# secondlaw-ai/skyrim

Hardware: AMD Instinct MI355X
Metric: 6-h forecast steps/sec on 721x1440 state, 1/2/4/8 MI355X; per-channel max rel-err vs ref (higher is better)
Workload: dtype f16; 1 GPU; Pangu 6-h autoregressive rollout, 721x1440x69 state (13 levels x 5 vars + 4 surface), random-init weights (64 M params), state resident in HBM, 1 ensemble membe; parallelism=single GPU, members=1, finite=True, rounding=compensated, term_plan=0x66f

## Files before the change

skyrim_amd/csrc/attention.hip:

```cpp
#include <cstdlib>
#include "gemm_dma.h"
#include "launchers.h"

namespace skp {

__device__ __forceinline__ int attn_key(int f, int row) {
    return f < 8 ? 32 * (f >> 1) + 8 * (row >> 2) + 4 * (f & 1) + (row & 3) : 128 + row;
}

__device__ __forceinline__ void attn_softmax_pv(f32x4 (&s)[9], const uint4 (&vf)[2][5], f32x4 (&o)[2], f32x4& osum) {
    typedef f16 T;
    const float LOG2E = 1.4426950408889634f;
    float mx = s[0][0];
#pragma unroll
    for (int f = 0; f < 9; ++f)
#pragma unroll
        for (int r = 0; r < 4; ++r) mx = fmaxf(mx, s[f][r]);
    mx = fmaxf(mx, __shfl_xor(mx, 16));
    mx = fmaxf(mx, __shfl_xor(mx, 32));
    const float mxl = mx * LOG2E;
#pragma unroll
    for (int f = 0; f < 9; ++f)
#pragma unroll
        for (int r = 0; r < 4; ++r) s[f][r] = __builtin_amdgcn_exp2f(__builtin_fmaf(s[f][r], LOG2E, -mxl));
    o[0] = f32x4{0.f, 0.f, 0.f, 0.f}; o[1] = f32x4{0.f, 0.f, 0.f, 0.f}; osum = f32x4{0.f, 0.f, 0.f, 0.f};
    const uint4 ones = make_uint4(0x3C003C00u, 0x3C003C00u, 0x3C003C00u, 0x3C003C00u);
#pragma unroll
    for (int kb = 0; kb < 5; ++kb) {
        float pv[8];
#pragma unroll
        for (int r = 0; r < 4; ++r) {
            pv[r] = s[2 * kb][r];
            pv[4 + r] = (kb < 4) ? s[(2 * kb + 1) % 9][r] : 0.f;
        }
        uint4 pf[1];
        split8<T, 1>(pv, pf);
#pragma unroll
        for (int df = 0; df < 2; ++df) o[df] = OpT<T>::mfma(as_v8<T>(vf[df][kb]), as_v8<T>(pf[0]), o[df]);
        osum = OpT<T>::mfma(as_v8<T>(ones), as_v8<T>(pf[0]), osum);
    }
}

constexpr int BT_ROW = 28, BT_COPY = 144 * BT_ROW + 120;

template <class TO, int NPL_O>
__global__ void __launch_bounds__(256) __attribute__((amdgpu_waves_per_eu(3, 3))) earth_attention2_kernel(const f16* __restrict__ q, const f16* __restrict__ k,
                                                              const f16* __restrict__ vt, const f16* __restrict__ bias_cmp, TO* __restrict__ out,
                                                              long long out_plane, int ld_out, int nW, int heads) {
    typedef f16 T;
    __shared__ __attribute__((aligned(16))) f16 tabs[4 * BT_COPY];
    const int lane = threadIdx.x & 63, wave = threadIdx.x >> 6;
    const int th = blockIdx.x;
    const int head = th % heads, type = th / heads;
    const int l15 = lane & 15, g = lane >> 4;
    {
        const f16* src = bias_cmp + (long long)th * 3456;
        for (int i = threadIdx.x; i < 3456; i += 256) {
            const int r = i / 24, e = i - 24 * r;
            const f16 v = src[i];
            if (e < 23) {
#pragma unroll
                for (int c = 0; c < 4; ++c) tabs[c * BT_COPY + r * BT_ROW + e + c] = v;
            }
        }
    }
    int koff[9];
#pragma unroll
    for (int f = 0; f < 9; ++f) {
        const int k0 = f < 8 ? 32 * (f >> 1) + 8 * g + 4 * (f & 1) : 128 + 4 * g;
        const int zk = k0 / 72, hk = (k0 / 12) % 6, wk0 = k0 % 12;
        koff[f] = 2 * ((2 * zk * 36 + 6 * hk) * BT_ROW + wk0);
    }
    __syncthreads();
    const char* tb = reinterpret_cast<const char*>(tabs);

    for (int wi = wave; wi < nW; wi += 4) {
        const int win = type * nW + wi;
        const long long base = (long long)win * heads + head;
        const T* qp = q + base * (WIN_TOKENS * HEAD_DIM) + l15 * HEAD_DIM + g * 8;
        const T* kp = k + base * (WIN_TOKENS * HEAD_DIM) + g * 8;
        const T* vp = vt + base * (WIN_TOKENS * HEAD_DIM) + (8 * (l15 >> 2) + (l15 & 3)) * WIN_TOKENS;

        uint4 kf[9];
#pragma unroll
        for (int f = 0; f < 9; ++f) kf[f] = *reinterpret_cast<const uint4*>(kp + attn_key(f, l15) * HEAD_DIM);
        uint4 vf[2][5];
#pragma unroll
        for (int df = 0; df < 2; ++df)
#pragma unroll
            for (int kb = 0; kb < 5; ++kb) {
                const T* s = vp + df * 4 * WIN_TOKENS;
                if (kb < 4) vf[df][kb] = *reinterpret_cast<const uint4*>(s + kb * 32 + g * 8);
                else { const uint2 lo = *reinterpret_cast<const uint2*>(s + 128 + g * 4); vf[df][kb] = make_uint4(lo.x, lo.y, 0, 0); }
            }
        uint4 qn = *reinterpret_cast<const uint4*>(qp);
#pragma unroll 1
        for (int qf = 0; qf < 9; ++qf) {
            const uint4 qv = qn;
            if (qf < 8) qn = *reinterpret_cast<const uint4*>(qp + (qf + 1) * 16 * HEAD_DIM);
            const int qi = 16 * qf + l15;
            const int zq = qi >= 72 ? 1 : 0, hq = (qi - 72 * zq) / 12, wq = qi - 72 * zq - 12 * hq;
            const int c = (wq + 1) & 3;
            const char* bq = tb + 2 * (c * BT_COPY + (zq * 36 + hq) * BT_ROW + (11 - wq) + c);
            uint2 bias[9];
#pragma unroll
            for (int f = 0; f < 9; ++f) bias[f] = *reinterpret_cast<const uint2*>(bq + koff[f]);

            f32x4 s[9];
#pragma unroll
            for (int f = 0; f < 9; ++f) {
                typedef f16 h4 __attribute__((ext_vector_type(4)));
                const h4 b = __builtin_bit_cast(h4, bias[f]);
                s[f] = OpT<T>::mfma(as_v8<T>(kf[f]), as_v8<T>(qv), f32x4{(float)b[0], (float)b[1], (float)b[2], (float)b[3]});
            }
            f32x4 o[2], osum;
            attn_softmax_pv(s, vf, o, osum);
            const float inv = __builtin_amdgcn_rcpf(osum[0]);
            TO* orow = out + blk_off((long long)win * WIN_TOKENS + qf * 16 + l15, head * HEAD_DIM, ld_out) + g * 8;
            const float y[8] = {o[0][0] * inv, o[0][1] * inv, o[0][2] * inv, o[0][3] * inv, o[1][0] * inv, o[1][1] * inv, o[1][2] * inv, o[1][3] * inv};
            store8_planes<TO, NPL_O>(orow, out_plane, y);
        }
    }
}


template <int C_, int PL_>
struct QaShape {
    static constexpr int C = C_, PL = PL_, KS = C / 32, NWAVES = 8, THREADS = 64 * NWAVES;
    static constexpr int BLK_KIB = KS * 2 * PL;
    static constexpr int W_BYTES = 3 * BLK_KIB * 1024;
    static constexpr int TAB_BYTES = (4 * BT_COPY * 2 + 1023) / 1024 * 1024;
    static constexpr int RING_BYTES = 6 * 1024;
    static constexpr int SMEM = W_BYTES + TAB_BYTES + 1024 + NWAVES * RING_BYTES;
    static_assert(SMEM <= 160 * 1024, "LDS");
};

struct QkvAttnArgs {
    const f16* xs;
    const int* widx;
    const f16* wf;
    const float* bias;
    const f16* bias_cmp;
    const f16* zrow;
    f16* out; long long out_plane;
    int nW, heads, types;
    float scale;
};

template <class S, int NPL_O>
__global__ void __launch_bounds__(S::THREADS) __attribute__((amdgpu_waves_per_eu(2, 2)))
qkv_attention_kernel(const QkvAttnArgs a) {
    typedef f16 T;
    constexpr int C = S::C, KS = S::KS, PL = S::PL;
    extern __shared__ __attribute__((aligned(16))) char smem[];
    char* wl = smem;
    f16* tabs = reinterpret_cast<f16*>(smem + S::W_BYTES);
    float* qb = reinterpret_cast<float*>(smem + S::W_BYTES + S::TAB_BYTES);
    const int tid = threadIdx.x, lane = tid & 63, l15 = lane & 15, g = lane >> 4;
    const int wave = __builtin_amdgcn_readfirstlane(tid >> 6);
    const int xcd = blockIdx.x & 7, slot = blockIdx.x >> 3;
    const int head = slot % a.heads, type = xcd + 8 * (slot / a.heads);
    if (type >= a.types) return;
    const int th = type * a.heads + head;
    {
        const unsigned lds_base = (unsigned)(size_t)smem;
#pragma unroll
        for (int which = 0; which < 3; ++which) {
            const f16* src = a.wf + ((long long)(which * a.heads + head) * S::BLK_KIB << 9) + lane * 8;
            for (int p = wave; p < S::BLK_KIB; p += S::NWAVES) glds16(src + (p << 9), lds_base + (unsigned)((which * S::BLK_KIB + p) << 10));
        }
        const f16* src = a.bias_cmp + (long long)th * 3456;
        constexpr int NT = (3456 + S::THREADS - 1) / S::THREADS;
        f16 tv[NT];
#pragma unroll
        for (int j = 0; j < NT; ++j) { const int i = tid + j * S::THREADS; tv[j] = src[i < 3456 ? i : 0]; }
#pragma unroll
        for (int j = 0; j < NT; ++j) {
            const int i = tid + j * S::THREADS;
            const int r = i / 24, e = i - 24 * r;
            if (i < 3456 && e < 23) {
#pragma unroll
                for (int c = 0; c < 4; ++c) tabs[c * BT_COPY + r * BT_ROW + e + c] = tv[j];
            }
        }
        if (tid < 96) qb[tid] = a.bias[(tid >> 5) * C + head * HEAD_DIM + (tid & 31)];
    }
    int koff[9];
#pragma unroll
    for (int f = 0; f < 9; ++f) {
        const int k0 = f < 8 ? 32 * (f >> 1) + 8 * g + 4 * (f & 1) : 128 + 4 * g;
        const int zk = k0 / 72, hk = (k0 / 12) % 6, wk0 = k0 % 12;
        koff[f] = 2 * ((2 * zk * 36 + 6 * hk) * BT_ROW + wk0);
    }
    int srcn[9];
    auto load_src = [&](int wi_) {
        const int w_ = type * a.nW + wi_;
#pragma unroll
        for (int f = 0; f < 9; ++f) srcn[f] = a.widx[w_ * WIN_TOKENS + attn_key(f, l15)];
    };
    load_src(wave < a.nW ? wave : 0);
    asm volatile("s_waitcnt vmcnt(0)" ::: "memory");
    __syncthreads();
    const char* tb = reinterpret_cast<const char*>(tabs);
    const char* wrd = wl + lane * 16;
    const unsigned ring_base = (unsigned)(size_t)smem + (unsigned)(S::W_BYTES + S::TAB_BYTES + 1024 + wave * S::RING_BYTES);
    const char* ring_rd = smem + S::W_BYTES + S::TAB_BYTES + 1024 + wave * S::RING_BYTES + lane * 16;

    for (int wi = wave; wi < a.nW; wi += S::NWAVES) {
        const int win = type * a.nW + wi;
        int src[9];
#pragma unroll
        for (int f = 0; f < 9; ++f) src[f] = srcn[f];
        uint4 qv[9], kf[9];
        uint2 vh[9][2];
        const T* xp[3];
        int xstep[3];
        auto point = [&](int tg_) {
#pragma unroll
            for (int i = 0; i < 3; ++i) {
                const int r = src[3 * tg_ + i];
                xp[i] = r >= 0 ? a.xs + blk_off(r, g * 8, C) : a.zrow;
                xstep[i] = r >= 0 ? 512 : 0;
            }
        };
        auto fetch = [&](int ks) {
#pragma unroll
            for (int i = 0; i < 3; ++i) glds16(xp[i] + ks * xstep[i], ring_base + (unsigned)(((ks & 1) * 3 + i) << 10));
        };
        point(0);
        fetch(0);
        fetch(1);
#pragma unroll
        for (int tg = 0; tg < 3; ++tg) {
            f32x4 qa[3][2], ka[3][2], va[3][2];
#pragma unroll
            for (int i = 0; i < 3; ++i)
#pragma unroll
                for (int n = 0; n < 2; ++n) { qa[i][n] = f32x4{0.f, 0.f, 0.f, 0.f}; ka[i][n] = f32x4{0.f, 0.f, 0.f, 0.f}; va[i][n] = f32x4{0.f, 0.f, 0.f, 0.f}; }
#pragma unroll 1
            for (int ks = 0; ks < KS; ++ks) {
                if (ks + 1 < KS) asm volatile("s_waitcnt vmcnt(3)" ::: "memory");
                else asm volatile("s_waitcnt vmcnt(0)" ::: "memory");
                uint4 xf[3];
#pragma unroll
                for (int i = 0; i < 3; ++i) xf[i] = *reinterpret_cast<const uint4*>(ring_rd + (((ks & 1) * 3 + i) << 10));
                if (ks + 2 < KS) {
                    asm volatile("s_waitcnt lgkmcnt(0)" ::: "memory");
                    fetch(ks + 2);
                }
#pragma unroll
                for (int which = 0; which < 3; ++which)
#pragma unroll
                    for (int n = 0; n < 2; ++n)
#pragma unroll
                        for (int p = PL - 1; p >= 0; --p) {
                            const uint4 w = *reinterpret_cast<const uint4*>(wrd + ((((which * KS + ks) * 2 + n) * PL + p) << 10));
#pragma unroll
                            for (int i = 0; i < 3; ++i) {
                                if (which == 0) qa[i][n] = OpT<T>::mfma(as_v8<T>(w), as_v8<T>(xf[i]), qa[i][n]);
                                else if (which == 1) ka[i][n] = OpT<T>::mfma(as_v8<T>(w), as_v8<T>(xf[i]), ka[i][n]);
                                else va[i][n] = OpT<T>::mfma(as_v8<T>(xf[i]), as_v8<T>(w), va[i][n]);
                            }
                        }
            }
            if (tg < 2) {
                point(tg + 1);
                fetch(0);
                fetch(1);
            }
            float bq[8], bk[8], bv[2];
#pragma unroll
            for (int i = 0; i < 8; ++i) { bq[i] = qb[8 * g + i]; bk[i] = qb[32 + 8 * g + i]; }
#pragma unroll
            for (int df = 0; df < 2; ++df) bv[df] = qb[64 + 8 * (l15 >> 2) + 4 * df + (l15 & 3)];
#pragma unroll
            for (int i = 0; i < 3; ++i) {
                const int f = 3 * tg + i;
                float v[8];
                uint4 o[1];
#pragma unroll
                for (int r = 0; r < 4; ++r) { v[r] = (qa[i][0][r] + bq[r]) * a.scale; v[4 + r] = (qa[i][1][r] + bq[4 + r]) * a.scale; }
                split8<T, 1>(v, o);
                qv[f] = o[0];
#pragma unroll
                for (int r = 0; r < 4; ++r) { v[r] = ka[i][0][r] + bk[r]; v[4 + r] = ka[i][1][r] + bk[4 + r]; }
                split8<T, 1>(v, o);
                kf[f] = o[0];
#pragma unroll
                for (int df = 0; df < 2; ++df) {
                    const float u[4] = {va[i][df][0] + bv[df], va[i][df][1] + bv[df], va[i][df][2] + bv[df], va[i][df][3] + bv[df]};
                    uint2 h[1];
                    split4<T, 1>(u, h);
                    vh[f][df] = h[0];
                }
            }
        }
        uint4 vf[2][5];
#pragma unroll
        for (int df = 0; df < 2; ++df) {
#pragma unroll
            for (int kb = 0; kb < 4; ++kb) vf[df][kb] = make_uint4(vh[2 * kb][df].x, vh[2 * kb][df].y, vh[2 * kb + 1][df].x, vh[2 * kb + 1][df].y);
            vf[df][4] = make_uint4(vh[8][df].x, vh[8][df].y, 0, 0);
        }
        if (wi + S::NWAVES < a.nW) load_src(wi + S::NWAVES);
#pragma unroll 1
        for (int qf = 0; qf < 9; ++qf) {
            const int qi = attn_key(qf, l15);
            const int zq = qi >= 72 ? 1 : 0, hq = (qi - 72 * zq) / 12, wq = qi - 72 * zq - 12 * hq;
            const int c = (wq + 1) & 3;
            const char* bqp = tb + 2 * (c * BT_COPY + (zq * 36 + hq) * BT_ROW + (11 - wq) + c);
            f32x4 s[9];
#pragma unroll
            for (int f = 0; f < 9; ++f) {
                typedef f16 h4 __attribute__((ext_vector_type(4)));
                const h4 b = __builtin_bit_cast(h4, *reinterpret_cast<const uint2*>(bqp + koff[f]));
                s[f] = OpT<T>::mfma(as_v8<T>(kf[f]), as_v8<T>(qv[qf]), f32x4{(float)b[0], (float)b[1], (float)b[2], (float)b[3]});
            }
            f32x4 o[2], osum;
            attn_softmax_pv(s, vf, o, osum);
            const float inv = __builtin_amdgcn_rcpf(osum[0]);
            T* orow = a.out + blk_off((long long)win * WIN_TOKENS + qi, head * HEAD_DIM, C) + g * 8;
            const float y[8] = {o[0][0] * inv, o[0][1] * inv, o[0][2] * inv, o[0][3] * inv, o[1][0] * inv, o[1][1] * inv, o[1][2] * inv, o[1][3] * inv};
            store8_planes<T, NPL_O>(orow, a.out_plane, y);
        }
    }
}

template <class S>
static hipError_t launch_qa(const QkvAttnArgs& a, int types, int out_planes, hipStream_t stream) {
    if (out_planes == 1) {
        auto kern = qkv_attention_kernel<S, 1>;
        hipError_t e = hipFuncSetAttribute(reinterpret_cast<const void*>(kern), hipFuncAttributeMaxDynamicSharedMemorySize, S::SMEM);
        if (e != hipSuccess) return e;
        hipLaunchKernelGGL(kern, dim3((unsigned)(8 * ((types + 7) / 8) * a.heads)), dim3(S::THREADS), S::SMEM, stream, a);
    } else {
        auto kern = qkv_attention_kernel<S, 2>;
        hipError_t e = hipFuncSetAttribute(reinterpret_cast<const void*>(kern), hipFuncAttributeMaxDynamicSharedMemorySize, S::SMEM);
        if (e != hipSuccess) return e;
        hipLaunchKernelGGL(kern, dim3((unsigned)(8 * ((types + 7) / 8) * a.heads)), dim3(S::THREADS), S::SMEM, stream, a);
    }
    return hipGetLastError();
}

hipError_t op_qkv_attention(const Geom& g, const BlockW<f16>& b, const int* widx, int res, const f16* Xs, const Work<PrecF16x3>& wk, hipStream_t s, int out_planes) {
    if (!b.bias_cmp || !(b.qkvh || b.qkvf)) return hipErrorInvalidValue;
    const int heads = res == 0 ? 6 : 12;
    QkvAttnArgs a{Xs, widx, b.qkvh ? b.qkvh : b.qkvf, b.qkv_b, b.bias_cmp, wk.zrow, wk.ao, wk.ao_plane, g.nW[res], heads, g.types[res], 0.17677669529663687f};
    if (b.qkvh) return res == 0 ? launch_qa<QaShape<192, 1>>(a, g.types[res], out_planes, s) : launch_qa<QaShape<384, 1>>(a, g.types[res], out_planes, s);
    if (res != 0) return hipErrorNotSupported;
    return launch_qa<QaShape<192, 2>>(a, g.types[res], out_planes, s);
}

template <class P>
hipError_t launch_attention(const AttnArgs<P>& a, hipStream_t stream) {
    constexpr int NPL_O = (P::NA > P::NW ? P::NA : P::NW);
    const int types = a.n_win / a.nW;
    if (a.out_planes == 1)
        hipLaunchKernelGGL((earth_attention2_kernel<typename P::T, 1>), dim3((unsigned)(types * a.heads)), dim3(256), 0, stream,
                           a.q, a.k, a.vt, a.bias_cmp, a.out, a.out_plane, a.ld_out, a.nW, a.heads);
    else
        hipLaunchKernelGGL((earth_attention2_kernel<typename P::T, NPL_O>), dim3((unsigned)(types * a.heads)), dim3(256), 0, stream,
                           a.q, a.k, a.vt, a.bias_cmp, a.out, a.out_plane, a.ld_out, a.nW, a.heads);
    return hipGetLastError();
}

template hipError_t launch_attention<PrecBF16x3>(const AttnArgs<PrecBF16x3>&, hipStream_t);
template hipError_t launch_attention<PrecF16x3>(const AttnArgs<PrecF16x3>&, hipStream_t);

}
```

Measured before the change: 70.19 steps/s.

## Make QKV attention kernel persistent with per-XCD type/head work scheduling

Replaces the one-block-per-(type,head) launch with a persistent grid sized to the CU count (a multiple of 8). Each block walks a static schedule of (type, head) units on its XCD. It reloads the head weights into LDS only when the head changes, and the relative-position bias table for every unit. This is meant to cut tail waves and repeated weight staging. It adds extra block-wide syncs between units and serialises work inside each block, which could lower parallelism if units are unevenly spread.

```diff
diff --git a/skyrim_amd/csrc/attention.hip b/skyrim_amd/csrc/attention.hip
--- a/skyrim_amd/csrc/attention.hip
+++ b/skyrim_amd/csrc/attention.hip
@@ -158,33 +158,28 @@
     float* qb = reinterpret_cast<float*>(smem + S::W_BYTES + S::TAB_BYTES);
     const int tid = threadIdx.x, lane = tid & 63, l15 = lane & 15, g = lane >> 4;
     const int wave = __builtin_amdgcn_readfirstlane(tid >> 6);
-    const int xcd = blockIdx.x & 7, slot = blockIdx.x >> 3;
-    const int head = slot % a.heads, type = xcd + 8 * (slot / a.heads);
-    if (type >= a.types) return;
-    const int th = type * a.heads + head;
-    {
-        const unsigned lds_base = (unsigned)(size_t)smem;
-#pragma unroll
-        for (int which = 0; which < 3; ++which) {
-            const f16* src = a.wf + ((long long)(which * a.heads + head) * S::BLK_KIB << 9) + lane * 8;
-            for (int p = wave; p < S::BLK_KIB; p += S::NWAVES) glds16(src + (p << 9), lds_base + (unsigned)((which * S::BLK_KIB + p) << 10));
-        }
-        const f16* src = a.bias_cmp + (long long)th * 3456;
-        constexpr int NT = (3456 + S::THREADS - 1) / S::THREADS;
-        f16 tv[NT];
-#pragma unroll
-        for (int j = 0; j < NT; ++j) { const int i = tid + j * S::THREADS; tv[j] = src[i < 3456 ? i : 0]; }
-#pragma unroll
-        for (int j = 0; j < NT; ++j) {
-            const int i = tid + j * S::THREADS;
-            const int r = i / 24, e = i - 24 * r;
-            if (i < 3456 && e < 23) {
-#pragma unroll
-                for (int c = 0; c < 4; ++c) tabs[c * BT_COPY + r * BT_ROW + e + c] = tv[j];
-            }
-        }
-        if (tid < 96) qb[tid] = a.bias[(tid >> 5) * C + head * HEAD_DIM + (tid & 31)];
-    }
+    const int xcd = blockIdx.x & 7, slot = blockIdx.x >> 3, P = gridDim.x >> 3;
+    const int n_x = xcd < a.types ? (a.types - xcd + 7) >> 3 : 0;
+    const int q = (n_x * a.heads + P - 1) / P, L = P / a.heads;
+    const int t_lanes = n_x < L * q ? n_x : L * q, n_rest = n_x - t_lanes;
+    auto sched_unit = [&](int i, int& type_, int& head_) -> bool {
+        if (i >= q) return false;
+        int ti;
+        if (slot < a.heads * L) {
+            head_ = slot % a.heads;
+            ti = slot / a.heads + i * L;
+            if (ti >= t_lanes) return false;
+        } else {
+            const int e = (slot - a.heads * L) * q + i;
+            if (e >= n_rest * a.heads) return false;
+            head_ = e / n_rest;
+            ti = t_lanes + e % n_rest;
+        }
+        type_ = xcd + 8 * ti;
+        return true;
+    };
+    int type, head;
+    if (!sched_unit(0, type, head)) return;
     int koff[9];
 #pragma unroll
     for (int f = 0; f < 9; ++f) {
@@ -193,20 +188,54 @@
         koff[f] = 2 * ((2 * zk * 36 + 6 * hk) * BT_ROW + wk0);
     }
     int srcn[9];
-    auto load_src = [&](int wi_) {
-        const int w_ = type * a.nW + wi_;
+    auto load_src = [&](int type_, int wi_) {
+        const int w_ = type_ * a.nW + wi_;
 #pragma unroll
         for (int f = 0; f < 9; ++f) srcn[f] = a.widx[w_ * WIN_TOKENS + attn_key(f, l15)];
     };
-    load_src(wave < a.nW ? wave : 0);
-    asm volatile("s_waitcnt vmcnt(0)" ::: "memory");
-    __syncthreads();
     const char* tb = reinterpret_cast<const char*>(tabs);
     const char* wrd = wl + lane * 16;
     const unsigned ring_base = (unsigned)(size_t)smem + (unsigned)(S::W_BYTES + S::TAB_BYTES + 1024 + wave * S::RING_BYTES);
     const char* ring_rd = smem + S::W_BYTES + S::TAB_BYTES + 1024 + wave * S::RING_BYTES + lane * 16;
 
-    for (int wi = wave; wi < a.nW; wi += S::NWAVES) {
+    int head_lds = -1;
+#pragma unroll 1
+    for (int ui = 0;; ++ui) {
+      int type_next = 0, head_next = 0;
+      const bool more = sched_unit(ui + 1, type_next, head_next);
+      load_src(type, wave < a.nW ? wave : 0);
+      if (ui > 0) __syncthreads();
+      int tid_u = (wave << 6) + (g << 4) + l15;
+      asm volatile("" : "+v"(tid_u));
+      if (head != head_lds) {
+        const unsigned lds_base = (unsigned)(size_t)smem;
+#pragma unroll
+        for (int which = 0; which < 3; ++which) {
+            const f16* src = a.wf + ((long long)(which * a.heads + head) * S::BLK_KIB << 9) + (tid_u & 63) * 8;
+            for (int p = wave; p < S::BLK_KIB; p += S::NWAVES) glds16(src + (p << 9), lds_base + (unsigned)((which * S::BLK_KIB + p) << 10));
+        }
+        if (tid_u < 96) qb[tid_u] = a.bias[(tid_u >> 5) * C + head * HEAD_DIM + (tid_u & 31)];
+        head_lds = head;
+      }
+      {
+        const f16* src = a.bias_cmp + (long long)(type * a.heads + head) * 3456;
+        constexpr int NT = (3456 + S::THREADS - 1) / S::THREADS;
+        f16 tv[NT];
+#pragma unroll
+        for (int j = 0; j < NT; ++j) { const int i = tid_u + j * S::THREADS; tv[j] = src[i < 3456 ? i : 0]; }
+#pragma unroll
+        for (int j = 0; j < NT; ++j) {
+            const int i = tid_u + j * S::THREADS;
+            const int r = i / 24, e = i - 24 * r;
+            if (i < 3456 && e < 23) {
+#pragma unroll
+                for (int c = 0; c < 4; ++c) tabs[c * BT_COPY + r * BT_ROW + e + c] = tv[j];
+            }
+        }
+      }
+      asm volatile("s_waitcnt vmcnt(0)" ::: "memory");
+      __syncthreads();
+      for (int wi = wave; wi < a.nW; wi += S::NWAVES) {
         const int win = type * a.nW + wi;
         int src[9];
 #pragma unroll
@@ -302,7 +331,7 @@
             for (int kb = 0; kb < 4; ++kb) vf[df][kb] = make_uint4(vh[2 * kb][df].x, vh[2 * kb][df].y, vh[2 * kb + 1][df].x, vh[2 * kb + 1][df].y);
             vf[df][4] = make_uint4(vh[8][df].x, vh[8][df].y, 0, 0);
         }
-        if (wi + S::NWAVES < a.nW) load_src(wi + S::NWAVES);
+        if (wi + S::NWAVES < a.nW) load_src(type, wi + S::NWAVES);
 #pragma unroll 1
         for (int qf = 0; qf < 9; ++qf) {
             const int qi = attn_key(qf, l15);
@@ -323,21 +352,43 @@
             const float y[8] = {o[0][0] * inv, o[0][1] * inv, o[0][2] * inv, o[0][3] * inv, o[1][0] * inv, o[1][1] * inv, o[1][2] * inv, o[1][3] * inv};
             store8_planes<T, NPL_O>(orow, a.out_plane, y);
         }
-    }
+      }
+      if (!more) break;
+      type = type_next; head = head_next;
+    }
+}
+
+static int qa_grid(hipError_t& e) {
+    static int grid[64] = {};
+    int dev = 0;
+    e = hipGetDevice(&dev);
+    if (e != hipSuccess) return 0;
+    if (dev < 0 || dev >= 64 || grid[dev] == 0) {
+        int cus = 0;
+        e = hipDeviceGetAttribute(&cus, hipDeviceAttributeMultiprocessorCount, dev);
+        if (e != hipSuccess) return 0;
+        const int n = cus >= 8 ? cus / 8 * 8 : 8;
+        if (dev < 0 || dev >= 64) return n;
+        grid[dev] = n;
+    }
+    return grid[dev];
 }
 
 template <class S>
 static hipError_t launch_qa(const QkvAttnArgs& a, int types, int out_planes, hipStream_t stream) {
+    hipError_t ge = hipSuccess;
+    const int grid = qa_grid(ge);
+    if (ge != hipSuccess) return ge;
     if (out_planes == 1) {
         auto kern = qkv_attention_kernel<S, 1>;
         hipError_t e = hipFuncSetAttribute(reinterpret_cast<const void*>(kern), hipFuncAttributeMaxDynamicSharedMemorySize, S::SMEM);
         if (e != hipSuccess) return e;
-        hipLaunchKernelGGL(kern, dim3((unsigned)(8 * ((types + 7) / 8) * a.heads)), dim3(S::THREADS), S::SMEM, stream, a);
+        hipLaunchKernelGGL(kern, dim3((unsigned)grid), dim3(S::THREADS), S::SMEM, stream, a);
     } else {
         auto kern = qkv_attention_kernel<S, 2>;
         hipError_t e = hipFuncSetAttribute(reinterpret_cast<const void*>(kern), hipFuncAttributeMaxDynamicSharedMemorySize, S::SMEM);
         if (e != hipSuccess) return e;
-        hipLaunchKernelGGL(kern, dim3((unsigned)(8 * ((types + 7) / 8) * a.heads)), dim3(S::THREADS), S::SMEM, stream, a);
+        hipLaunchKernelGGL(kern, dim3((unsigned)grid), dim3(S::THREADS), S::SMEM, stream, a);
     }
     return hipGetLastError();
 }
```

Measured after the change: 69.86 steps/s. Within noise of the previous version (-0.5%).
